# davrempe/contact-human-dynamics

Measured on NVIDIA H100. Metric: optimised frames/sec (batched phys-optim), higher is better.
Workload: dtype f64

## Files before the change

### contact-human-dynamics_b200/csrc/chd_kkt.cu

```cuda
#include <cuda_runtime.h>

#include "chd_block.cuh"
#include "chd_eval.cuh"
#include "chd_kkt_tiles.cuh"

__device__ __forceinline__ void chd_hess_sample(const ChdCtx& c, const ChdKT& K, const int* vk, int s, const ChdSpl* P, const double* sign, int np,
                                                int deriv, double wgt, int lane, double* ws) {
  const bool tau = c.opt_dur && s >= 2 && deriv == 0;
  if (lane < 28) {
    const int pa = lane / 14, q = lane % 14;
    double v0 = 0.0, v1 = 0.0, v2 = 0.0;
    int ia = -1;
    if (pa < np) {
      if (q < 12) {
        const int va = P[pa].var[q];
        const double wa = sign[pa] * chd_slot_w(P[pa], deriv, q);
        if (va >= 0 && wa != 0.0) {
          ia = vk[va];
          v0 = q % 3 == 0 ? wa : 0.0, v1 = q % 3 == 1 ? wa : 0.0, v2 = q % 3 == 2 ? wa : 0.0;
        }
      } else if (tau) {
        ChdTau u;
        chd_spl_tau(c, s, s - 2, P[pa], u);
        const int var = q == 12 ? u.va : u.vb;
        const double* dv = q == 12 ? u.da : u.db;
        if (var >= 0) ia = vk[var], v0 = sign[pa] * dv[0], v1 = sign[pa] * dv[1], v2 = sign[pa] * dv[2];
      }
    }
    ws[lane * 4 + 0] = (double)ia, ws[lane * 4 + 1] = v0, ws[lane * 4 + 2] = v1, ws[lane * 4 + 3] = v2;
  }
  __syncwarp();
  const int ne = np * 14;
  for (int idx = lane; idx < ne * ne; idx += 32) {
    const int a = idx / ne, bq = idx - a * ne;
    const int ia = (int)ws[a * 4], ib = (int)ws[bq * 4];
    if (ia < 0 || ib < 0 || ia < ib) continue;
    const double v = ws[a * 4 + 1] * ws[bq * 4 + 1] + ws[a * 4 + 2] * ws[bq * 4 + 2] + ws[a * 4 + 3] * ws[bq * 4 + 3];
    if (v != 0.0) chd_kadd(K, ia, ib, wgt * v);
  }
  __syncwarp();
}

__device__ void chd_hess_build(const ChdDev& D, int b, const ChdStageDev& sg, double* base, int part, int nparts) {
  const int tid = threadIdx.x, nt = blockDim.x;
  const ChdSeq* h = D.seq + b;
  ChdKT K;
  chd_kt_init(D, h, base, K);
  K.ovf = &D.ipm[b].band_ovf;
  const double sf = D.ipm[b].sf;
  const int* vk = D.var_kkt + (size_t)b * D.n_max;
  ChdCtx c;
  chd_make_ctx(D, b, D.x + (size_t)b * D.n_max, c);
  c.dyn = D.ipm[b].dyn;
  c.opt_dur = sg.opt_dur;
  const int n_ee = h->n_ee, nsp = 2 + n_ee, F = h->F, ns = h->n_smooth;
  __shared__ double s_hws[CHD_THREADS / 32][28 * 4];
  const int lane = tid & 31, warp = tid >> 5, nwarp = nt >> 5;
  for (int it = part * nwarp + warp; it < nsp * F; it += nparts * nwarp) {
    const int s = it / F, i = it % F, cls = s < 2 ? s : 2;
    ChdSpl P[2];
    double sgn[2] = {1.0, -1.0};
    chd_spl_at(c, s, c.t_data[i], P[1]);
    if (sg.w_data[cls] != 0.0) chd_hess_sample(c, K, vk, s, P + 1, sgn, 1, 0, sf * sg.w_data[cls], lane, s_hws[warp]);
    if (i < ns && (sg.w_vel[cls] != 0.0 || sg.w_acc[cls] != 0.0)) {
      chd_spl_at(c, s, c.t_data[i] + h->dt, P[0]);
      if (sg.w_vel[cls] != 0.0) chd_hess_sample(c, K, vk, s, P, sgn, 2, 0, sf * sg.w_vel[cls], lane, s_hws[warp]);
      if (sg.w_acc[cls] != 0.0) chd_hess_sample(c, K, vk, s, P, sgn, 2, 1, sf * sg.w_acc[cls], lane, s_hws[warp]);
    }
  }
  if (part == 0)
    for (int i = K.Na + tid; i < K.Np; i += nt) *chd_kdiag(K, i, true) = 1.0;
  if (part == 0 && !sg.opt_dur && h->dur_band)
    for (int i = tid; i < h->n_dur; i += nt) *chd_kdiag(K, vk[h->dur_xoff[0] + i], true) = 1.0;
  if (part == 0 && sg.opt_dur && sg.w_dur != 0.0) {
    for (int ee = 0; ee < n_ee; ++ee)
      for (int k = tid; k < h->n_phases[ee] - 1; k += nt) {
        const int i = vk[h->dur_xoff[ee] + k];
        chd_kadd(K, i, i, sf * sg.w_dur);
        if (k > 0) {
          const int j = vk[h->dur_xoff[ee] + k - 1];
          chd_kadd(K, j, j, sf * sg.w_dur);
          chd_kadd(K, i, j, -sf * sg.w_dur);
        }
      }
  }
}
__device__ void chd_hess_clear(const ChdDev& D, int b, double* base, int part, int nparts) {
  const size_t cnt2 = D.kstride / 2, per = (cnt2 + nparts - 1) / nparts;
  const size_t lo = (size_t)part * per, hi = lo + per < cnt2 ? lo + per : cnt2;
  double2* dst = reinterpret_cast<double2*>(base);
  for (size_t i = lo + threadIdx.x; i < hi; i += blockDim.x) dst[i] = make_double2(0.0, 0.0);
}
__device__ void chd_rhs_clear(const ChdDev& D, int b) {
  const size_t go = (size_t)b * (D.Na_max + D.nb_max);
  for (int i = threadIdx.x; i < D.Na_max + D.nb_max; i += blockDim.x) D.rhs0[go + i] = 0.0, D.rhs1[go + i] = 0.0;
}

__global__ void __launch_bounds__(CHD_THREADS) chd_k_hess_dur(ChdDev D) {
  const int b = blockIdx.y;
  const ChdIpm& I = D.ipm[b];
  if (I.phase != CHD_PH_RUN || !I.kw_req) return;
  const ChdStageDev sg = D.stages[I.stage];
  if (!sg.opt_dur) return;
  chd_hess_build(D, b, sg, D.Kwork + (size_t)b * D.kstride, blockIdx.x, gridDim.x);
}
__global__ void __launch_bounds__(128) chd_k_hess_fin(ChdDev D, int mode) {
  const int b = blockIdx.x;
  ChdIpm& I = D.ipm[b];
  double* base;
  if (mode == 0) {
    if (I.phase != CHD_PH_BEGIN) return;
    base = D.Kbase + (size_t)b * D.kstride;
  } else {
    if (I.phase != CHD_PH_RUN || !I.kw_req || !D.stages[I.stage].opt_dur) return;
    base = D.Kwork + (size_t)b * D.kstride;
  }
  const ChdSeq* h = D.seq + b;
  const int* vk = D.var_kkt + (size_t)b * D.n_max;
  ChdKT K;
  chd_kt_init(D, h, base, K);
  unsigned char* un = D.unobs + (size_t)b * D.n_max;
  const int mot_lo = h->sp_xoff[2], mot_hi = h->sp_xoff[2 + h->n_ee];
  for (int i = mot_lo + threadIdx.x; i < mot_hi; i += blockDim.x) {
    const int k = vk[i];
    un[i] = k >= 0 && *chd_kdiag(K, k) <= CHD_UNOBS_EPS;
  }
  __syncthreads();
  if (mode == 0 && threadIdx.x == 0) I.phase = CHD_PH_RUN;
}

__device__ __forceinline__ void chd_curv_rows(const ChdDev& D, int b, const ChdKT& K, const ChdStageDev& sg, int wid, int nw, int lane,
                                              double* ws) {
  const ChdSeq* h = D.seq + b;
  const size_t ro = (size_t)b * D.m_max, vo = (size_t)b * D.n_max;
  const int* vk = D.var_kkt + vo;
  ChdCtx c;
  chd_make_ctx(D, b, D.x + vo, c);
  c.dyn = D.ipm[b].dyn;
  c.opt_dur = sg.opt_dur;
  for (int si = 0; si < h->nsets; ++si) {
    const ChdSet st = c.sets[si];
    if (!(sg.set_mask & CHD_MASK(st.type))) continue;
    if (st.type != CHD_SET_ROM && st.type != CHD_SET_HEEL) continue;
    const int nslot = st.type == CHD_SET_ROM ? 38 : 28;
    for (int k = wid; k < st.nitems; k += nw) {
      const int R = st.row0 + k;
      const double yc = D.sc[ro + R] * D.y[ro + R];
      if (!(yc > CHD_CURV_MIN)) continue;
      const double t = c.t_rom[k];
      ChdSpl P0, P1, P2;
      double dRh[3][3];
      if (st.type == CHD_SET_ROM) {
        chd_spl_at(c, 0, t, P0);
        chd_spl_at(c, 1, t, P1);
        chd_spl_at(c, chd_sp_motion(st.a), t, P2);
        double e[3];
        chd_spl_val(c, P1, 0, e);
        ChdTrig tr;
        chd_trig(e, tr);
        const double* hip = chd_hip(c, st.a, t);
        for (int j = 0; j < 3; ++j) {
          double Dj[9];
          chd_dR(tr, j, Dj);
          chd_mv(Dj, hip, dRh[j]);
        }
      } else {
        chd_spl_at(c, chd_sp_motion(st.a), t, P0);
        chd_spl_at(c, chd_sp_motion(st.b), t, P1);
      }
      ChdTau ua, ub;
      ua.va = ua.vb = ub.va = ub.vb = -1;
      if (c.opt_dur) {
        if (st.type == CHD_SET_ROM) chd_spl_tau(c, chd_sp_motion(st.a), st.a, P2, ua);
        else chd_spl_tau(c, chd_sp_motion(st.a), st.a, P0, ua), chd_spl_tau(c, chd_sp_motion(st.b), st.b, P1, ub);
      }
      const int nnode = st.type == CHD_SET_ROM ? 36 : 24;
      for (int a = lane; a < nslot; a += 32) {
        if (a >= nnode) {
          const int t4 = a - nnode;
          const ChdTau& u = t4 < 2 ? ua : ub;
          const int var = (t4 & 1) ? u.vb : u.va;
          const double* dv = (t4 & 1) ? u.db : u.da;
          const int ia = var >= 0 ? vk[var] : -1;
          ws[a * 5 + 0] = (double)ia;
          ws[a * 5 + 1] = ia >= 0 ? (t4 < 2 ? 1.0 : -1.0) : 0.0;
          ws[a * 5 + 2] = ia >= 0 ? dv[0] : 0.0, ws[a * 5 + 3] = ia >= 0 ? dv[1] : 0.0, ws[a * 5 + 4] = ia >= 0 ? dv[2] : 0.0;
          continue;
        }
        const int ba = a / 12, qa = a % 12, da = qa % 3;
        const ChdSpl& Pa = ba == 0 ? P0 : (ba == 1 ? P1 : P2);
        const int va = Pa.var[qa];
        const int ia = va >= 0 ? vk[va] : -1;
        double sgn, v3[3] = {da == 0 ? 1.0 : 0.0, da == 1 ? 1.0 : 0.0, da == 2 ? 1.0 : 0.0};
        if (st.type == CHD_SET_ROM) {
          sgn = ba == 2 ? 1.0 : -1.0;
          if (ba == 1) v3[0] = dRh[da][0], v3[1] = dRh[da][1], v3[2] = dRh[da][2];
        } else {
          sgn = ba == 0 ? 1.0 : -1.0;
        }
        ws[a * 5 + 0] = (double)ia;
        ws[a * 5 + 1] = ia >= 0 ? sgn * chd_slot_w(Pa, 0, qa) : 0.0;
        ws[a * 5 + 2] = v3[0], ws[a * 5 + 3] = v3[1], ws[a * 5 + 4] = v3[2];
      }
      __syncwarp();
      for (int idx = lane; idx < nslot * nslot; idx += 32) {
        const int a = idx / nslot, bq = idx - a * nslot;
        const double wa = ws[a * 5 + 1], wb = ws[bq * 5 + 1];
        if (wa == 0.0 || wb == 0.0) continue;
        const int ia = (int)ws[a * 5], ib = (int)ws[bq * 5];
        if (ia < ib) continue;
        const double dotv = ws[a * 5 + 2] * ws[bq * 5 + 2] + ws[a * 5 + 3] * ws[bq * 5 + 3] + ws[a * 5 + 4] * ws[bq * 5 + 4];
        if (dotv != 0.0) chd_kadd(K, ia, ib, yc * wa * wb * dotv);
      }
      __syncwarp();
    }
  }
}

__global__ void __launch_bounds__(256) chd_k_hess_zero(ChdDev D) {
  const int b = blockIdx.y;
  if (D.ipm[b].phase != CHD_PH_BEGIN) return;
  chd_hess_clear(D, b, D.Kbase + (size_t)b * D.kstride, blockIdx.x, gridDim.x);
  chd_hess_clear(D, b, D.Kwork + (size_t)b * D.kstride, blockIdx.x, gridDim.x);
  if (blockIdx.x == 0) chd_rhs_clear(D, b);
}
__global__ void __launch_bounds__(256, 2) chd_k_hess_base(ChdDev D) {
  __shared__ double s_ws[8][192];
  const int b = blockIdx.y;
  if (D.ipm[b].phase != CHD_PH_BEGIN) return;
  const ChdStageDev sg = D.stages[D.ipm[b].stage];
  ChdKT K;
  chd_kt_init(D, D.seq + b, D.Kwork + (size_t)b * D.kstride, K);
  K.ovf = &D.ipm[b].band_ovf;
  const int warp = threadIdx.x >> 5, nwarp = blockDim.x >> 5;
  chd_curv_rows(D, b, K, sg, blockIdx.x * nwarp + warp, gridDim.x * nwarp, threadIdx.x & 31, s_ws[warp]);
  chd_hess_build(D, b, sg, D.Kbase + (size_t)b * D.kstride, blockIdx.x, gridDim.x);
  chd_hess_build(D, b, sg, D.Kwork + (size_t)b * D.kstride, blockIdx.x, gridDim.x);
}

__device__ __forceinline__ void chd_assemble(const ChdDev& D, int b, const ChdKT& K, double delta_w, double sf, int t0, int tstep,
                                             double* g0, double* g1) {
  const ChdSeq* h = D.seq + b;
  const int n = D.stages[D.ipm[b].stage].opt_dur ? h->n : h->n - h->n_dur;
  const int m = h->m, Na = K.Na;
  const size_t ro = (size_t)b * D.m_max, vo = (size_t)b * D.n_max;
  const int* rf = D.rflag + ro;
  const int* vk = D.var_kkt + vo;
  const int* rk = D.row_kkt + ro;
  const int* ep = D.ent_ptr + (size_t)b * (D.m_max + 1);
  const int* ec = D.ent_col + (size_t)b * D.slots_max;
  const double* Jv = D.Jv + (size_t)b * D.slots_max;
  const double* grad = D.grad + vo;
  auto gidx = [&](int kk) { return kk < Na ? kk : D.Na_max + (kk - Na); };
  auto g_add = [&](int kk, double v0, double v1) {
    atomicAdd(g0 + gidx(kk), v0);
    if (v1 != 0.0) atomicAdd(g1 + gidx(kk), v1);
  };
  const unsigned char* unobs = D.unobs + vo;
  for (int i = t0; i < n; i += tstep) {
    const int k = vk[i];
    if (k < 0) continue;
    if (unobs[i]) chd_kadd(K, k, k, CHD_DW_UNOBS);
    chd_kadd(K, k, k, delta_w);
    g_add(k, -sf * grad[i], 0.0);
  }
  for (int r = t0; r < m; r += tstep) {
    const int f = rf[r];
    const int k = rk[r];
    if (!(f & CHD_ROW_ACTIVE)) {
      if (k >= 0) chd_kadd(K, k, k, -1.0);
      continue;
    }
    const double sc = D.sc[ro + r];
    const int e0 = ep[r], e1 = ep[r + 1];
    if (k >= 0) {
      double diag = -CHD_DELTA_C, rr0, rr1 = 0.0;
      if (f & CHD_ROW_EQ) {
        rr0 = -(sc * D.g[ro + r] - D.dL[ro + r]);
      } else {
        const double s = D.s[ro + r];
        const double gapL = (f & CHD_ROW_HASL) ? s - D.dL[ro + r] : 1.0, gapU = (f & CHD_ROW_HASU) ? D.dU[ro + r] - s : 1.0;
        const double Sig = ((f & CHD_ROW_HASL) ? D.zL[ro + r] / gapL : 0.0) + ((f & CHD_ROW_HASU) ? D.zU[ro + r] / gapU : 0.0);
        diag -= 1.0 / Sig;
        rr0 = -(sc * D.g[ro + r] - s) + D.y[ro + r] / Sig;
        rr1 = (((f & CHD_ROW_HASL) ? 1.0 / gapL : 0.0) - ((f & CHD_ROW_HASU) ? 1.0 / gapU : 0.0)) / Sig;
      }
      chd_kadd(K, k, k, diag);
      g_add(k, rr0, rr1);
      const double ys = sc * D.y[ro + r];
      for (int e = e0; e < e1; ++e) {
        const int col = ec[e];
        if (col < 0) continue;
        const int kc = vk[col];
        if (kc < 0) continue;
        const double jv = Jv[e];
        if (jv == 0.0) continue;
        chd_kadd(K, k, kc, sc * jv);
        g_add(kc, -ys * jv, 0.0);
      }
    } else {
      const double s = D.s[ro + r];
      const double gapL = (f & CHD_ROW_HASL) ? s - D.dL[ro + r] : 1.0, gapU = (f & CHD_ROW_HASU) ? D.dU[ro + r] - s : 1.0;
      const double Sig = ((f & CHD_ROW_HASL) ? D.zL[ro + r] / gapL : 0.0) + ((f & CHD_ROW_HASU) ? D.zU[ro + r] / gapU : 0.0);
      const double coef0 = Sig * (sc * D.g[ro + r] - s);
      const double beta = ((f & CHD_ROW_HASL) ? 1.0 / gapL : 0.0) - ((f & CHD_ROW_HASU) ? 1.0 / gapU : 0.0);
      for (int ea = e0; ea < e1; ++ea) {
        const int ca = ec[ea];
        if (ca < 0) continue;
        const int ka = vk[ca];
        if (ka < 0) continue;
        const double va = sc * Jv[ea];
        if (va == 0.0) continue;
        g_add(ka, -va * coef0, va * beta);
        for (int eb = e0; eb < e1; ++eb) {
          const int cb = ec[eb];
          if (cb < 0) continue;
          const int kb = vk[cb];
          if (kb < 0 || ka < kb) continue;
          const double vb = sc * Jv[eb];
          if (vb != 0.0) chd_kadd(K, ka, kb, Sig * va * vb);
        }
      }
    }
  }
}

struct ChdKktCtx {
  int b, tid, nt, lane, warp, nwarp;
  ChdIpm* I;
  ChdStageDev sg;
  const ChdSeq* h;
  int n, m, n_act, Qs, Q, nbt, nbp8, nbl, nbc, NBR, nbt_s;
  size_t ro, vo, n_even, xs_len, win_region;
  const int *rf, *vk, *rk, *ep, *ec;
  const double *Jv, *grad;
  ChdKT K;
  double *red, *cc, *ypan, *xpan, *dinv, *win, *bwin, *vecn, *xs, *xs2;
  double sf, mu, tau, delta_w;
  bool polish;
};

template <bool WS>
__device__ __forceinline__ void chd_kkt_ctx_init(const ChdDev& D, ChdIpm& I, ChdKktCtx& c) {
  extern __shared__ double sm[];
  const int b = blockIdx.x;
  c.b = b, c.I = &I;
  c.sg = D.stages[I.stage];
  const ChdSeq* h = c.h = D.seq + b;
  c.n = h->n, c.m = h->m, c.tid = threadIdx.x, c.nt = blockDim.x;
  c.lane = c.tid & 31, c.warp = c.tid >> 5, c.nwarp = c.nt >> 5;
  c.ro = (size_t)b * D.m_max, c.vo = (size_t)b * D.n_max;
  c.rf = D.rflag + c.ro;
  c.vk = D.var_kkt + c.vo;
  c.rk = D.row_kkt + c.ro;
  c.ep = D.ent_ptr + (size_t)b * (D.m_max + 1);
  c.ec = D.ent_col + (size_t)b * D.slots_max;
  c.Jv = D.Jv + (size_t)b * D.slots_max;
  c.grad = D.grad + c.vo;
  ChdKT& K = c.K;
  chd_kt_init(D, h, D.Kwork + (size_t)b * D.kstride, K);
  K.ovf = &I.band_ovf;
  if (!c.sg.opt_dur) K.q = D.Qfix - 1;
  c.n_act = c.sg.opt_dur ? c.n : c.n - h->n_dur;
  c.Qs = K.Q, c.Q = c.sg.opt_dur ? K.Q : D.Qfix, c.nbt = K.nbt, c.nbp8 = K.nbp8, c.nbl = c.sg.opt_dur ? h->nb : h->nb_fix, c.nbc = K.nbc;
  c.NBR = c.nbl, c.nbt_s = (c.nbl + 1 + 7) >> 3;
  c.n_even = (size_t)((D.n_max + 1) & ~1), c.xs_len = (size_t)(8 * D.nbc_max + c.nbp8);
  double* gs = WS ? nullptr : D.scratch + (size_t)b * D.scratch_stride;
  c.red = sm;
  c.cc = c.red + CHD_KKT_THREADS;
  c.ypan = c.cc + c.nbp8 * c.nbp8;
  c.xpan = c.ypan + (c.Q + c.nbt) * 64;
  c.dinv = c.ypan + D.pan_doubles;
  c.win_region = (size_t)D.win_tiles * 64 + (size_t)c.Qs * c.nbt * 64;
  c.win = WS ? c.dinv + 16 : gs + c.n_even + c.xs_len + 8 * (size_t)D.nbc_max;
  c.bwin = c.win + (size_t)D.win_tiles * 64;
  c.vecn = WS ? c.win + c.win_region - c.n_even : gs;
  c.xs = WS ? c.vecn - c.xs_len : c.vecn + c.n_even;
  c.xs2 = WS ? c.ypan : c.xs + c.xs_len;
  c.sf = I.sf;
}

__device__ __forceinline__ bool chd_kkt_errors(const ChdDev& D, ChdKktCtx& c, int& s_fail) {
  ChdIpm& I = *c.I;
  const int b = c.b, tid = c.tid, nt = c.nt, n = c.n, m = c.m, n_act = c.n_act;
  const size_t ro = c.ro, vo = c.vo;
  const int *rf = c.rf, *vk = c.vk, *ep = c.ep, *ec = c.ec;
  const double *Jv = c.Jv, *grad = c.grad, sf = c.sf;
  double* red = c.red;
  double mu = I.mu;
  const int* erow = D.ent_row + (size_t)b * D.slots_max;
  const int* cptr = D.col_ptr + (size_t)b * (D.n_max + 1);
  const int* cent = D.col_ent + (size_t)b * D.slots_max;
  double* rowv = D.dy + ro;
  double a_ysum = 0, a_zsum = 0, a_cviol = 0, a_theta = 0, a_rs = 0, a_cmax = -INFINITY, a_cmin = INFINITY, a_violu = 0;
  for (int r = tid; r < m; r += nt) {
    const int f = rf[r];
    if (!(f & CHD_ROW_ACTIVE)) {
      rowv[r] = 0.0;
      continue;
    }
    const double sc = D.sc[ro + r], gval = D.g[ro + r], d = sc * gval, y = D.y[ro + r];
    a_ysum += fabs(y);
    a_violu = fmax(a_violu, fmax(D.row_lo[ro + r] - gval, gval - D.row_hi[ro + r]));
    rowv[r] = sc * y;
    if (f & CHD_ROW_EQ) {
      const double re = d - D.dL[ro + r];
      a_cviol = fmax(a_cviol, fabs(re));
      a_theta += fabs(re);
    } else {
      const double s = D.s[ro + r], ri = d - s, zL = D.zL[ro + r], zU = D.zU[ro + r];
      a_cviol = fmax(a_cviol, fabs(ri));
      a_theta += fabs(ri);
      a_rs = fmax(a_rs, fabs(-y - zL + zU));
      a_zsum += zL + zU;
      if (f & CHD_ROW_HASL) { const double cp = (s - D.dL[ro + r]) * zL; a_cmax = fmax(a_cmax, cp); a_cmin = fmin(a_cmin, cp); }
      if (f & CHD_ROW_HASU) { const double cp = (D.dU[ro + r] - s) * zU; a_cmax = fmax(a_cmax, cp); a_cmin = fmin(a_cmin, cp); }
    }
  }
  __syncthreads();
  double a_dual = 0;
  if (!I.dyn) {
    for (int i = tid; i < n_act; i += nt) {
      double v = sf * grad[i];
      for (int t = cptr[i]; t < cptr[i + 1]; ++t) {
        const int e = cent[t];
        v += rowv[erow[e]] * Jv[e];
      }
      if (vk[i] >= 0) a_dual = fmax(a_dual, fabs(v));
    }
  } else {
    double* jty = D.jty + vo;
    for (int i = tid; i < n; i += nt) jty[i] = 0.0;
    __syncthreads();
    for (int r = tid; r < m; r += nt) {
      const double ys = rowv[r];
      if (ys == 0.0) continue;
      for (int e = ep[r]; e < ep[r + 1]; ++e) {
        const int col = ec[e];
        if (col >= 0 && Jv[e] != 0.0) atomicAdd(jty + col, ys * Jv[e]);
      }
    }
    __syncthreads();
    for (int i = tid; i < n_act; i += nt)
      if (vk[i] >= 0) a_dual = fmax(a_dual, fabs(sf * grad[i] + jty[i]));
  }
  const double ysum = chd_block_sum(a_ysum, red), zsum = chd_block_sum(a_zsum, red);
  const double cviol = chd_block_max(a_cviol, red), theta = chd_block_sum(a_theta, red);
  const double dual_inf = fmax(chd_block_max(a_dual, red), chd_block_max(a_rs, red));
  const double cmax = chd_block_max(a_cmax, red), cmin = chd_block_min(a_cmin, red);
  const double violu = fmax(chd_block_max(a_violu, red), 0.0);
  const int nbnd = I.n_bounds;
  const double s_d = fmax(CHD_S_MAX, (ysum + zsum) / fmax((double)(I.m_act + nbnd), 1.0)) / CHD_S_MAX;
  const double s_c = fmax(CHD_S_MAX, zsum / fmax((double)nbnd, 1.0)) / CHD_S_MAX;
  auto compl_err = [&](double mm) { return nbnd > 0 ? fmax(fabs(cmax - mm), fabs(cmin - mm)) : 0.0; };
  const double E0 = fmax(fmax(dual_inf / s_d, cviol), compl_err(0.0) / s_c);
  const double dual_u = dual_inf / sf, compl_u = compl_err(0.0) / sf;
  bool done = false;
  int new_status = 1;
  if (E0 <= CHD_TOL && violu <= CHD_CONSTR_VIOL_TOL && dual_u <= CHD_DUAL_INF_TOL && compl_u <= CHD_COMPL_INF_TOL) new_status = 0, done = true;
  else if (I.iter >= I.max_iter) new_status = -1, done = true;
  if (!done) {
    const double mu_min = fmin(CHD_TOL, CHD_COMPL_INF_TOL) / (CHD_KAPPA_EPS + 1.0);
    while (true) {
      const double Emu = fmax(fmax(dual_inf / s_d, cviol), compl_err(mu) / s_c);
      if (Emu <= CHD_KAPPA_EPS * mu && mu > mu_min) mu = fmax(mu_min, fmin(CHD_KAPPA_MU * mu, pow(mu, CHD_THETA_MU)));
      else break;
    }
  }
  __syncthreads();
  if (tid == 0) {
    I.f = D.cost[2 * b];
    I.E0 = E0, I.viol_u = violu, I.dual_u = dual_u, I.compl_u = compl_u;
    I.status = new_status;
    s_fail = 0;
    if (done) chd_stage_advance(D, I, new_status, c.sg.snap_after);
    if (!done) {
      I.mu = mu;
      I.tau = fmax(CHD_TAU_MIN, 1.0 - mu);
      if (I.iter == 0) I.theta_max = 1e4 * fmax(1.0, theta), I.theta_min = 1e-4 * fmax(1.0, theta), I.theta_ref = theta;
      if (mu != I.mu_filter) I.nfilt = 0, I.mu_filter = mu;
      I.theta0 = theta;
    }
  }
  if (done) return true;
  c.mu = mu;
  c.tau = fmax(CHD_TAU_MIN, 1.0 - mu);
  c.polish = E0 <= CHD_TOL && dual_u <= CHD_DUAL_INF_TOL && compl_u <= CHD_COMPL_INF_TOL && violu > CHD_CONSTR_VIOL_TOL &&
             I.delta_w < CHD_DW_POLISH;
  c.delta_w = c.polish ? CHD_DW_POLISH : I.delta_w;
  return false;
}

__device__ __forceinline__ void chd_kkt_assemble(const ChdDev& D, const ChdKktCtx& c) {
  const ChdIpm& I = *c.I;
  const ChdKT& K = c.K;
  const int tid = c.tid, nt = c.nt, n_act = c.n_act, nbl = c.nbl, nbt = c.nbt, nbp8 = c.nbp8, NBR = c.NBR, Na = K.Na;
  const int* vk = c.vk;
  const double mu = c.mu;
  if (c.polish) {
    const double extra = c.delta_w - I.delta_w;
    for (int i = tid; i < n_act; i += nt)
      if (vk[i] >= 0) chd_kadd(K, vk[i], vk[i], extra);
  }
  const double* r0 = D.rhs0 + (size_t)c.b * (D.Na_max + D.nb_max);
  const double* r1 = D.rhs1 + (size_t)c.b * (D.Na_max + D.nb_max);
  for (int i = tid; i < K.Np; i += nt)
    K.bord[((size_t)(i >> 3) * nbt + (NBR >> 3)) * 64 + (NBR & 7) * 8 + (i & 7)] = i < Na ? r0[i] + mu * r1[i] : 0.0;
  for (int i = tid; i < nbl; i += nt) K.corn[(size_t)NBR * nbp8 + i] = r0[D.Na_max + i] + mu * r1[D.Na_max + i];
}

template <class BandTile, class BordTile>
__device__ __forceinline__ void chd_kkt_update_block(const ChdKktCtx& c, const int* gi, const int* gj, const bool* vi, const bool* vj, bool diag,
                                                     int GB, const BandTile& band_tile, const BordTile& bord_tile) {
  const int lane = c.lane;
  const double2 z = make_double2(0.0, 0.0);
  double2 xf[2], yf[2];
#pragma unroll
  for (int a = 0; a < 2; ++a) {
    xf[a] = vi[a] ? *reinterpret_cast<const double2*>(c.xpan + gi[a] * 64 + 2 * lane) : z;
    yf[a] = vj[a] ? *reinterpret_cast<const double2*>(c.ypan + gj[a] * 64 + 2 * lane) : z;
  }
  double* Cp[4];
  double2 cv[4];
#pragma unroll
  for (int t = 0; t < 4; ++t) {
    const int a = t & 1, cl = t >> 1;
    bool ok = vi[a] && vj[cl] && !(diag && a == 0 && cl == 1);
    ok = ok && !(gi[a] == 0 && gj[cl] == 0);
    Cp[t] = nullptr;
    if (ok) {
      if (gi[a] < GB) Cp[t] = band_tile(gi[a], gj[cl]) + (lane >> 2) * 8 + 2 * (lane & 3);
      else if (gj[cl] < GB) Cp[t] = bord_tile(gi[a] - GB, gj[cl]) + (lane >> 2) * 8 + 2 * (lane & 3);
      else Cp[t] = c.cc + (size_t)((gi[a] - GB) * 8 + (lane >> 2)) * c.nbp8 + (gj[cl] - GB) * 8 + 2 * (lane & 3);
    }
    cv[t] = ok ? *reinterpret_cast<const double2*>(Cp[t]) : z;
  }
  const double2 xt = make_double2(-xf[0].x, -xf[0].y), xb = make_double2(-xf[1].x, -xf[1].y);
#pragma unroll
  for (int cl = 0; cl < 2; ++cl) chd_mma_16x8x8(cv[2 * cl], cv[2 * cl + 1], xt, xb, yf[cl]);
#pragma unroll
  for (int t = 0; t < 4; ++t)
    if (Cp[t]) *reinterpret_cast<double2*>(Cp[t]) = cv[t];
}

template <class BandTile, class BordTile>
__device__ __forceinline__ void chd_kkt_update_compact(const ChdKktCtx& c, const unsigned short* s_pairs, unsigned char* cmp, const int* gnz,
                                                       int GB, int Gm, int tq, const BandTile& band_tile, const BordTile& bord_tile) {
  const int lane = c.lane, warp = c.warp;
  int na;
  {
    const int g1 = lane + 32;
    const bool act0 = lane < Gm && (lane >= GB || lane < tq) && gnz[lane];
    const bool act1 = g1 < Gm && (g1 >= GB || g1 < tq) && gnz[g1 < 96 ? g1 : 0];
    const unsigned m0 = __ballot_sync(0xffffffffu, act0), m1 = __ballot_sync(0xffffffffu, act1);
    const unsigned below = (1u << lane) - 1u;
    const int n0 = __popc(m0);
    na = n0 + __popc(m1);
    if (act0) cmp[__popc(m0 & below)] = (unsigned char)lane;
    if (act1) cmp[n0 + __popc(m1 & below)] = (unsigned char)g1;
    __syncwarp();
  }
  const int step = c.nwarp - 1;
  const int nb2 = (na + 1) >> 1, nblk = nb2 * (nb2 + 1) / 2;
  for (int p = warp - 1; p < nblk; p += step) {
    const int bi = s_pairs[p] >> 8, bj = s_pairs[p] & 255;
    const int i1 = 2 * bi + 1, j1 = 2 * bj + 1;
    const int gi[2] = {cmp[2 * bi], cmp[i1 & 63]}, gj[2] = {cmp[2 * bj], cmp[j1 & 63]};
    const bool vi[2] = {true, i1 < na}, vj[2] = {true, j1 < na};
    chd_kkt_update_block(c, gi, gj, vi, vj, bi == bj, GB, band_tile, bord_tile);
  }
}

template <class BandTile, class BordTile>
__device__ __forceinline__ void chd_kkt_update_wide(const ChdKktCtx& c, const unsigned short* s_pairs, const int* gnz, int GB, int Gm,
                                                    int tq, const BandTile& band_tile, const BordTile& bord_tile) {
  auto live = [&](int g) { return g < Gm && (g >= GB || g < tq) && gnz[g]; };
  const int nb2 = (Gm + 1) >> 1, nblk = nb2 * (nb2 + 1) / 2;
  for (int p = c.warp - 1; p < nblk; p += c.nwarp - 1) {
    const int bi = s_pairs[p] >> 8, bj = s_pairs[p] & 255;
    const int gi[2] = {2 * bi, 2 * bi + 1}, gj[2] = {2 * bj, 2 * bj + 1};
    const bool vi[2] = {live(gi[0]), live(gi[1])}, vj[2] = {live(gj[0]), live(gj[1])};
    if (!(vi[0] || vi[1]) || !(vj[0] || vj[1])) continue;
    chd_kkt_update_block(c, gi, gj, vi, vj, bi == bj, GB, band_tile, bord_tile);
  }
}

template <bool WS>
__device__ __forceinline__ void chd_kkt_factor(const ChdKktCtx& c, int& s_fail) {
  const ChdKT& K = c.K;
  const int tid = c.tid, nt = c.nt, lane = c.lane, warp = c.warp, nwarp = c.nwarp;
  const int Qs = c.Qs, Q = c.Q, nbt = c.nbt, nbp8 = c.nbp8, nbc = c.nbc, nbt_s = c.nbt_s;
  double *cc = c.cc, *ypan = c.ypan, *xpan = c.xpan, *dinv = c.dinv, *win = c.win, *bwin = c.bwin;
  for (int i = tid; i < nbp8 * nbp8; i += nt) cc[i] = K.corn[i];
  if (WS) {
    for (int idx = tid; idx < Q * Q * 64; idx += nt) {
      const int e = idx & 63, pr = idx >> 6, J = pr / Q, t = pr % Q;
      if (J + t < Q && J < nbc && J + t < nbc) win[chd_win_slot(J + t, J, Q) * 64 + e] = K.band[((size_t)J * Qs + t) * 64 + e];
    }
    for (int idx = tid; idx < Q * nbt * 64; idx += nt) {
      const int J = idx / (nbt * 64);
      if (J < nbc) bwin[idx] = K.bord[(size_t)J * nbt * 64 + idx % (nbt * 64)];
    }
  }
  __syncthreads();
  __shared__ int s_rs[2][96];
  __shared__ int s_gnz[2][96];
  constexpr int kPairs = WS ? 3000 : CHD_KKT_GROUPS_MAX * (CHD_KKT_GROUPS_MAX + 1) / 2;
  __shared__ unsigned short s_pairs[kPairs];
  __shared__ unsigned char s_cmp[CHD_KKT_THREADS / 32][64];
  __shared__ __align__(16) double s_winv[2][64];
#ifdef CHD_PROFILE
  __shared__ unsigned long long s_upd_end;
  double prof_diag = 0.0, prof_upd = 0.0;
  if (tid == 0) s_upd_end = 0;
#endif
  const int GB = K.q, Gm = K.q + nbt_s, nb2 = (Gm + 1) >> 1, npairs = nb2 * (nb2 + 1) / 2;
  for (int p = tid; p < npairs && p < kPairs; p += nt) {
    int gi = (int)((sqrt(8.0 * p + 1.0) - 1.0) * 0.5);
    while (gi * (gi + 1) / 2 > p) --gi;
    while ((gi + 1) * (gi + 2) / 2 <= p) ++gi;
    s_pairs[p] = (unsigned short)((gi << 8) | (p - gi * (gi + 1) / 2));
  }
  auto tri = [](int a_, int b_) { return a_ > b_ ? a_ * (a_ + 1) / 2 + b_ : b_ * (b_ + 1) / 2 + a_; };
  for (int g = tid; g < GB; g += nt) s_rs[0][g] = (1 + g) % Q;
  for (int g = tid; g < 96; g += nt) s_gnz[0][g] = 0, s_gnz[1][g] = 0;
  if (warp == 0) {
    const bool ok = chd_tile_ldl(WS ? win : K.band, dinv, s_winv[0], lane);
    if (!ok && lane == 0) s_fail = 1;
  }
  __syncthreads();
  int kslot = 0, cur = 0;
  for (int Kc = 0; Kc < nbc; ++Kc, cur ^= 1) {
    const int tq = min(K.q, nbc - 1 - Kc);
    const int* rs = s_rs[cur];
    auto band_tile = [&](int gi, int gj) -> double* {
      return WS ? win + (size_t)tri(rs[gi], rs[gj]) * 64 : K.band + ((size_t)(Kc + 1 + gj) * Qs + (gi - gj)) * 64;
    };
    auto bord_tile = [&](int bi, int gj) -> double* {
      return WS ? bwin + ((size_t)rs[gj] * nbt + bi) * 64 : K.bord + ((size_t)(Kc + 1 + gj) * nbt + bi) * 64;
    };
    double* Tkk = WS ? win + (size_t)tri(kslot, kslot) * 64 : K.band + (size_t)Kc * Qs * 64;
    double* Bk = WS ? bwin + (size_t)kslot * nbt * 64 : K.bord + (size_t)Kc * nbt * 64;
    const double* dv = dinv + 8 * cur;
    {
      const double* wv = s_winv[cur];
      const int r = lane >> 2, k = lane & 3, ng = tq + nbt_s;
      const double2 wf = *reinterpret_cast<const double2*>(wv + 2 * lane);
      const double d0 = dv[2 * k], d1 = dv[2 * k + 1];
      const int f0 = r * 8 + chd_frag_col(2 * k), f1 = r * 8 + chd_frag_col(2 * k + 1);
      for (int g0 = 2 * warp; g0 < ng; g0 += 2 * nwarp) {
        double2 a[2], y[2];
#pragma unroll
        for (int h = 0; h < 2; ++h) {
          const int g = g0 + h;
          const double* A = g < tq ? (WS ? win + (size_t)tri(rs[g], kslot) * 64 : K.band + ((size_t)Kc * Qs + 1 + g) * 64) : Bk + (g - tq) * 64;
          a[h] = g < ng ? make_double2(A[r * 8 + k], A[r * 8 + k + 4]) : make_double2(0.0, 0.0);
          y[h] = make_double2(0.0, 0.0);
        }
        chd_mma_16x8x8(y[0], y[1], a[0], a[1], wf);
#pragma unroll
        for (int h = 0; h < 2; ++h) {
          const int g = g0 + h;
          if (g >= ng) break;
          const bool band_t = g < tq;
          const int pg = band_t ? g : GB + (g - tq);
          const double x0 = y[h].x * d0, x1 = y[h].y * d1;
          ypan[pg * 64 + f0] = y[h].x, ypan[pg * 64 + f1] = y[h].y;
          xpan[pg * 64 + f0] = x0, xpan[pg * 64 + f1] = x1;
          double* G = band_t ? K.band + ((size_t)Kc * Qs + 1 + g) * 64 : K.bord + ((size_t)Kc * nbt + (g - tq)) * 64;
          *reinterpret_cast<double2*>(G + r * 8 + 2 * k) = make_double2(x0, x1);
          const bool nz = __any_sync(0xffffffffu, x0 != 0.0 || x1 != 0.0);
          if (lane == 0 && nz) s_gnz[cur][pg] = 1;
        }
      }
    }
    if (WS)
      for (int e = tid; e < 64; e += nt) K.band[(size_t)Kc * Qs * 64 + e] = Tkk[e];
    __syncthreads();
    const int In = Kc + Q;
#ifdef CHD_PROFILE
    const long long tc0 = clock64();
#endif
    if (WS && In < nbc) {
      for (int idx = tid - 32; idx < Q * 32 + nbt_s * 32; idx += nt - 32) {
        if (idx < 0) break;
        const int tile = idx >> 5, off = (idx & 31) * 2;
        if (tile < Q) {
          const int J = tile < GB ? Kc + 1 + tile : In;
          double* dst = tile < GB ? win + (size_t)tri(kslot, rs[tile]) * 64 : Tkk;
          chd_copy16(dst + off, K.band + ((size_t)J * Qs + (In - J)) * 64 + off, WS);
        } else {
          chd_copy16(Bk + (tile - Q) * 64 + off, K.bord + (size_t)In * nbt * 64 + (tile - Q) * 64 + off, WS);
        }
      }
    }
    if (warp == 0) {
      if (tq >= 1) {
        double* Tn = band_tile(0, 0);
        chd_tile_sub_xyT(Tn, xpan, ypan, lane);
        __syncwarp();
        const bool ok = chd_tile_ldl(Tn, dinv + 8 * (cur ^ 1), s_winv[cur ^ 1], lane);
        if (!ok && lane == 0) s_fail = 1;
      }
#ifdef CHD_PROFILE
      if (lane == 0) prof_diag += (double)(clock64() - tc0);
#endif
    } else {
      if (warp == 1) {
        for (int g = lane; g < GB; g += 32) {
          int v = kslot + 2 + g;
          while (v >= Q) v -= Q;
          s_rs[cur ^ 1][g] = v;
        }
        for (int g = lane; g < Gm; g += 32) s_gnz[cur ^ 1][g] = 0;
      }
      if (!WS && Gm > 64) chd_kkt_update_wide(c, s_pairs, s_gnz[cur], GB, Gm, tq, band_tile, bord_tile);
      else chd_kkt_update_compact(c, s_pairs, s_cmp[warp], s_gnz[cur], GB, Gm, tq, band_tile, bord_tile);
#ifdef CHD_PROFILE
      if (lane == 0) atomicMax(&s_upd_end, (unsigned long long)clock64());
#endif
    }
    chd_copy_wait(WS);
    __syncthreads();
#ifdef CHD_PROFILE
    if (tid == 0) prof_upd += (double)((long long)s_upd_end - tc0);
#endif
    kslot = kslot + 1 == Q ? 0 : kslot + 1;
  }
#ifdef CHD_PROFILE
  if (tid == 0) c.I->prof[6] += prof_diag, c.I->prof[7] += prof_upd;
#endif
}

__device__ __forceinline__ void chd_kkt_border(const ChdDev& D, const ChdKktCtx& c, int& s_fail) {
  const int tid = c.tid, nt = c.nt, lane = c.lane, warp = c.warp, nbl = c.nbl, nbp8 = c.nbp8, NBR = c.NBR, Na = c.K.Na;
  double* cc = c.cc;
  for (int k = 0; k < nbl; ++k) {
    const double dk = cc[k * nbp8 + k];
    if (tid == 0 && !(dk > 0.0 && isfinite(dk))) s_fail = 1;
    __syncthreads();
    const double ik = 1.0 / dk;
    const int rem = nbl - k - 1;
    for (int idx = tid; idx < rem * rem; idx += nt) {
      const int i = k + 1 + idx / rem, j = k + 1 + idx % rem;
      if (j <= i) cc[i * nbp8 + j] -= cc[i * nbp8 + k] * ik * cc[j * nbp8 + k];
    }
    for (int j = k + 1 + tid; j < nbl; j += nt) cc[NBR * nbp8 + j] -= cc[j * nbp8 + k] * ik * cc[NBR * nbp8 + k];
    __syncthreads();
  }
  double* xb = c.xs + 8 * D.nbc_max;
  if (warp == 0) {
    for (int j = lane; j < nbl; j += 32) xb[j] = cc[NBR * nbp8 + j];
    __syncwarp();
    for (int k = nbl - 1; k >= 0; --k) {
      const double xk = xb[k] / cc[k * nbp8 + k];
      __syncwarp();
      for (int j = lane; j < k; j += 32) xb[j] -= cc[k * nbp8 + j] * xk;
      if (lane == 0) xb[k] = xk;
      __syncwarp();
    }
  }
  __syncthreads();
  for (int i = tid; i < nbl; i += nt) D.sol[(size_t)c.b * (D.Na_max + D.nb_max) + Na + i] = xb[i];
}

template <bool WS>
__device__ __forceinline__ void chd_kkt_backsub(const ChdDev& D, const ChdKktCtx& c) {
  const ChdKT& K = c.K;
  const int tid = c.tid, nt = c.nt, lane = c.lane, warp = c.warp, Q = c.Q, Qs = c.Qs, nbt = c.nbt, nbl = c.nbl, nbc = c.nbc;
  const int NBR = c.NBR, Na = K.Na;
  double *xs = c.xs, *sol = D.sol + (size_t)c.b * (D.Na_max + D.nb_max);
  const double* xb = xs + 8 * D.nbc_max;
  double* accv = c.xs2;
  for (int i = tid; i < K.Np; i += nt) {
    const double* bt = K.bord + (size_t)(i >> 3) * nbt * 64 + (i & 7);
    double v = bt[NBR * 8];
    for (int q2 = 0; q2 < nbl; ++q2) v -= bt[q2 * 8] * xb[q2];
    accv[i] = v;
  }
  const int per = Q * 64;
  const int R = max(1, (int)((c.win_region - (WS ? c.n_even + c.xs_len : 0)) / 64) / (2 * Q));
  double* stg = c.win;
  auto stage_chunk = [&](int Ktop, int buf, int t0, int tstep) {
    for (int idx = t0; idx < R * Q * 32; idx += tstep) {
      const int rr = idx / (Q * 32), rem = idx - rr * (Q * 32);
      const int Kr = Ktop - rr;
      if (Kr < 0) break;
      const int tile = rem >> 5, off = (rem & 31) * 2;
      const int J = tile == 0 ? Kr : Kr - tile;
      if (J < 0) continue;
      chd_copy16(stg + ((size_t)buf * R + rr) * per + tile * 64 + off, K.band + ((size_t)J * Qs + (Kr - J)) * 64 + off, WS);
    }
  };
  stage_chunk(nbc - 1, 0, tid, nt);
  chd_copy_wait(WS);
  __syncthreads();
  int buf = 0;
  for (int Ktop = nbc - 1; Ktop >= 0; Ktop -= R, buf ^= 1) {
    if (warp != 0) {
      stage_chunk(Ktop - R, buf ^ 1, tid - 32, nt - 32);
    } else {
      for (int rr = 0; rr < R && Ktop - rr >= 0; ++rr) {
        const int Kc = Ktop - rr;
        const double* T0 = stg + ((size_t)buf * R + rr) * per;
        double xk[8];
#pragma unroll
        for (int cl = 7; cl >= 0; --cl) {
          double v = accv[Kc * 8 + cl];
#pragma unroll
          for (int p = 7; p > cl; --p) v -= T0[p * 8 + cl] * xk[p];
          xk[cl] = v;
        }
        if (lane < 8) {
          const int gi = Kc * 8 + lane;
          double v = xk[0];
#pragma unroll
          for (int cl = 1; cl < 8; ++cl) v = lane == cl ? xk[cl] : v;
          xs[gi] = v;
          if (gi < Na) sol[gi] = v;
        }
        const int nrow = min(K.q, Kc);
        for (int idx = lane; idx < nrow * 8; idx += 32) {
          const int g = idx >> 3, cl = idx & 7;
          const double* T = T0 + (g + 1) * 64;
          double v = 0.0;
#pragma unroll
          for (int r = 0; r < 8; ++r) v += T[r * 8 + cl] * xk[r];
          accv[(Kc - 1 - g) * 8 + cl] -= v;
        }
        __syncwarp();
      }
    }
    chd_copy_wait(WS);
    __syncthreads();
  }
}

__device__ __forceinline__ bool chd_kkt_no_step(const ChdDev& D, const ChdKktCtx& c, const int& s_fail) {
  ChdIpm& I = *c.I;
  const int tid = c.tid, nt = c.nt, n = c.n, m = c.m;
  const size_t ro = c.ro, vo = c.vo;
  if (I.band_ovf) {
    __syncthreads();
    if (tid == 0) I.status = -2, chd_stage_advance(D, I, -2, c.sg.snap_after);
    return true;
  }
  if (s_fail) {
    if (tid == 0) {
      I.delta_w = fmin(fmax(I.delta_w * 100.0, 1e-4), CHD_DW_MAX * 10);
      I.a_pr = 0.0, I.a_du = 0.0, I.dphi = 0.0;
      I.ls_fail += 1;
      I.step_ready = 1;
      I.kw_req = 1;
      if (I.delta_w > CHD_DW_MAX) I.status = -2, chd_stage_advance(D, I, -2, c.sg.snap_after);
    }
    for (int i = tid; i < n; i += nt) D.dx[vo + i] = 0.0;
    for (int r = tid; r < m; r += nt) D.ds[ro + r] = 0.0, D.dy[ro + r] = 0.0, D.dzL[ro + r] = 0.0, D.dzU[ro + r] = 0.0;
    return true;
  }
  return false;
}

__device__ __forceinline__ void chd_kkt_recover(const ChdDev& D, const ChdKktCtx& c) {
  ChdIpm& I = *c.I;
  const ChdSeq* h = c.h;
  const int b = c.b, tid = c.tid, nt = c.nt, n = c.n, m = c.m, n_act = c.n_act;
  const size_t ro = c.ro, vo = c.vo;
  const int *rf = c.rf, *vk = c.vk, *rk = c.rk, *ep = c.ep, *ec = c.ec;
  const double *Jv = c.Jv, *grad = c.grad, *sol = D.sol + (size_t)c.b * (D.Na_max + D.nb_max), sf = c.sf, mu = c.mu, tau = c.tau;
  double *vecn = c.vecn, *red = c.red;
  double* dx = D.dx + vo;
  for (int i = tid; i < n; i += nt) {
    const int k = vk[i];
    const double v = (k >= 0 && i < n_act) ? sol[k] : 0.0;
    dx[i] = v;
    vecn[i] = v;
  }
  __syncthreads();
  if (c.sg.opt_dur) {
    for (int ee = 0; ee < h->n_ee; ++ee)
      for (int k = 1 + tid; k < h->n_phases[ee] - 1; k += nt) dx[h->dur_xoff[ee] + k] = vecn[h->dur_xoff[ee] + k] - vecn[h->dur_xoff[ee] + k - 1];
  }
  double a_pr = 1.0, a_du = 1.0, a_dphi = 0.0, a_phi = 0.0;
  for (int i = tid; i < n; i += nt) a_dphi += sf * grad[i] * vecn[i];
  for (int r = tid; r < m; r += nt) {
    const int f = rf[r];
    if (!(f & CHD_ROW_ACTIVE)) continue;
    if (f & CHD_ROW_EQ) {
      D.dy[ro + r] = sol[rk[r]];
      D.ds[ro + r] = 0.0;
      continue;
    }
    const double sc = D.sc[ro + r], s = D.s[ro + r];
    double Jdx = 0.0;
    for (int e = ep[r]; e < ep[r + 1]; ++e) {
      const int col = ec[e];
      if (col >= 0) Jdx += Jv[e] * vecn[col];
    }
    const double riq = sc * D.g[ro + r] - s;
    const double ds = sc * Jdx + riq;
    const bool hl = f & CHD_ROW_HASL, hu = f & CHD_ROW_HASU;
    const double gapL = hl ? s - D.dL[ro + r] : 1.0, gapU = hu ? D.dU[ro + r] - s : 1.0;
    const double zL = D.zL[ro + r], zU = D.zU[ro + r];
    const double sigL = hl ? zL / gapL : 0.0, sigU = hu ? zU / gapU : 0.0;
    const double bvec = (hl ? mu / gapL : 0.0) - (hu ? mu / gapU : 0.0);
    const double dy = (sigL + sigU) * ds - D.y[ro + r] - bvec;
    const double dzL = hl ? mu / gapL - zL - sigL * ds : 0.0;
    const double dzU = hu ? mu / gapU - zU + sigU * ds : 0.0;
    D.ds[ro + r] = ds, D.dy[ro + r] = dy, D.dzL[ro + r] = dzL, D.dzU[ro + r] = dzU;
    if (hl && ds < 0) a_pr = fmin(a_pr, -tau * gapL / ds);
    if (hu && ds > 0) a_pr = fmin(a_pr, tau * gapU / ds);
    if (hl && dzL < 0) a_du = fmin(a_du, -tau * zL / dzL);
    if (hu && dzU < 0) a_du = fmin(a_du, -tau * zU / dzU);
    if (hl) a_dphi -= mu * ds / gapL, a_phi -= mu * log(gapL);
    if (hu) a_dphi += mu * ds / gapU, a_phi -= mu * log(gapU);
  }
  a_pr = chd_block_min(a_pr, red);
  a_du = chd_block_min(a_du, red);
  const double dphi = chd_block_sum(a_dphi, red);
  const double phib = chd_block_sum(a_phi, red);
  if (tid == 0) {
    I.a_pr = a_pr, I.a_du = a_du, I.dphi = dphi;
    I.phi0 = sf * D.cost[2 * b] + phib;
    I.step_ready = 1;
    I.kw_req = 1;
  }
}

template <bool WS>
__device__ __forceinline__ void chd_kkt_body(const ChdDev& D) {
  __shared__ int s_fail;
  ChdIpm& I = D.ipm[blockIdx.x];
  if (I.phase != CHD_PH_RUN) return;
  ChdKktCtx c;
  chd_kkt_ctx_init<WS>(D, I, c);
#ifdef CHD_PROFILE
  long long tk0 = clock64();
#define CHD_PROF(slot) do { __syncthreads(); if (c.tid == 0) { long long t_ = clock64(); I.prof[slot] += (double)(t_ - tk0); tk0 = t_; } } while (0)
#else
#define CHD_PROF(slot) do { } while (0)
#endif
  if (chd_kkt_errors(D, c, s_fail)) return;
  CHD_PROF(0);
  chd_kkt_assemble(D, c);
  __syncthreads();
  CHD_PROF(1);
  chd_kkt_factor<WS>(c, s_fail);
  CHD_PROF(2);
  chd_kkt_border(D, c, s_fail);
  CHD_PROF(3);
  chd_kkt_backsub<WS>(D, c);
  CHD_PROF(4);
  if (chd_kkt_no_step(D, c, s_fail)) return;
  __syncthreads();
  chd_kkt_recover(D, c);
  CHD_PROF(5);
}
#undef CHD_PROF

__global__ void __launch_bounds__(256) chd_k_kcopy(ChdDev D) {
  const int b = blockIdx.y;
  if (!D.ipm[b].kw_req) return;
  if (blockIdx.x == 0) chd_rhs_clear(D, b);
  if (D.stages[D.ipm[b].stage].opt_dur && D.ipm[b].phase == CHD_PH_RUN) {
    chd_hess_clear(D, b, D.Kwork + (size_t)b * D.kstride, blockIdx.x, gridDim.x);
    return;
  }
  const size_t cnt2 = D.kstride / 2, per = (cnt2 + gridDim.x - 1) / gridDim.x;
  const size_t lo = (size_t)blockIdx.x * per, hi = lo + per < cnt2 ? lo + per : cnt2;
  const double2* src = reinterpret_cast<const double2*>(D.Kbase + (size_t)b * D.kstride);
  double2* dst = reinterpret_cast<double2*>(D.Kwork + (size_t)b * D.kstride);
  const size_t nt = blockDim.x;
  size_t i = lo + threadIdx.x;
  for (; i + 3 * nt < hi; i += 4 * nt) {
    const double2 v0 = src[i], v1 = src[i + nt], v2 = src[i + 2 * nt], v3 = src[i + 3 * nt];
    dst[i] = v0, dst[i + nt] = v1, dst[i + 2 * nt] = v2, dst[i + 3 * nt] = v3;
  }
  for (; i < hi; i += nt) dst[i] = src[i];
}

__global__ void __launch_bounds__(256) chd_k_curv(ChdDev D) {
  __shared__ double s_ws[8 * 192];
  const int b = blockIdx.y;
  const ChdIpm& I = D.ipm[b];
  if (!I.kw_req || I.phase != CHD_PH_RUN) return;
  ChdKT K;
  chd_kt_init(D, D.seq + b, D.Kwork + (size_t)b * D.kstride, K);
  K.ovf = &D.ipm[b].band_ovf;
  const int warp = threadIdx.x >> 5, lane = threadIdx.x & 31;
  chd_curv_rows(D, b, K, D.stages[I.stage], blockIdx.x * 8 + warp, gridDim.x * 8, lane, s_ws + warp * 192);
}

__global__ void __launch_bounds__(256) chd_k_asm(ChdDev D) {
  const int b = blockIdx.y;
  const ChdIpm& I = D.ipm[b];
  if (I.phase != CHD_PH_RUN) return;
  ChdKT K;
  chd_kt_init(D, D.seq + b, D.Kwork + (size_t)b * D.kstride, K);
  K.ovf = &D.ipm[b].band_ovf;
  if (!D.stages[I.stage].opt_dur) K.q = D.Qfix - 1;
  const size_t go = (size_t)b * (D.Na_max + D.nb_max);
  chd_assemble(D, b, K, I.delta_w, I.sf, blockIdx.x * blockDim.x + threadIdx.x, gridDim.x * blockDim.x, D.rhs0 + go, D.rhs1 + go);
}

__global__ void __launch_bounds__(256) chd_k_fp64_peak(int mode, int iters, double* sink) {
  const double s = 1.0 + 1e-9 * threadIdx.x;
  double2 a[8];
#pragma unroll
  for (int i = 0; i < 8; ++i) a[i] = make_double2(0.5 + i, 1.5 + i);
  if (mode == 0) {
    for (int it = 0; it < iters; ++it) {
#pragma unroll
      for (int i = 0; i < 8; ++i) a[i].x = fma(a[i].x, s, 1e-3);
    }
  } else {
    const double2 x = make_double2(s, s), y = make_double2(1.0 - 1e-9 * threadIdx.x, 1.0);
    for (int it = 0; it < iters; ++it) {
#pragma unroll
      for (int i = 0; i < 4; ++i) chd_mma_16x8x8(a[2 * i], a[2 * i + 1], x, x, y);
    }
  }
  double t = 0;
#pragma unroll
  for (int i = 0; i < 8; ++i) t += a[i].x + a[i].y;
  if (t == 123.456) sink[threadIdx.x] = t;
}

__global__ void __launch_bounds__(CHD_KKT_THREADS) chd_k_kkt(ChdDev D) { chd_kkt_body<true>(D); }
__global__ void __launch_bounds__(CHD_KKT_THREADS) chd_k_kkt_gwin(ChdDev D) { chd_kkt_body<false>(D); }
```

Before: 13770.

## Block the border Cholesky into 8x8 tiles with tensor-core MMA and pad backsub staging

Replaces the scalar right-looking border factorisation, which needs two block barriers per column, with a blocked LDL over 8x8 tiles. Warp 0 factors the next diagonal tile while the other warps apply the trailing update, and the panel solve uses f64 MMA fragments. The border back-solve now expects unit-diagonal factors. Backsub staging tiles are padded to a 72-double stride to cut shared-memory bank conflicts, and the off-diagonal accumulation processes four tile rows per lane for more ILP. The new code depends on extra context buffers (ypan, xpan, dinv, red, nwarp) and adds more shared-memory use and complexity.

```diff
diff --git a/contact-human-dynamics_b200/csrc/chd_kkt.cu b/contact-human-dynamics_b200/csrc/chd_kkt.cu
--- a/contact-human-dynamics_b200/csrc/chd_kkt.cu
+++ b/contact-human-dynamics_b200/csrc/chd_kkt.cu
@@ -733,35 +733,100 @@
 }
 
 __device__ __forceinline__ void chd_kkt_border(const ChdDev& D, const ChdKktCtx& c, int& s_fail) {
-  const int tid = c.tid, nt = c.nt, lane = c.lane, warp = c.warp, nbl = c.nbl, nbp8 = c.nbp8, NBR = c.NBR, Na = c.K.Na;
-  double* cc = c.cc;
-  for (int k = 0; k < nbl; ++k) {
-    const double dk = cc[k * nbp8 + k];
-    if (tid == 0 && !(dk > 0.0 && isfinite(dk))) s_fail = 1;
+  const int tid = c.tid, lane = c.lane, warp = c.warp, nwarp = c.nwarp, nbl = c.nbl, nbp8 = c.nbp8, NBR = c.NBR, Na = c.K.Na;
+  double *cc = c.cc, *ypan = c.ypan, *xpan = c.xpan, *dinv = c.dinv;
+  double* winv = c.red;
+  double* Td = c.red + 128;
+  const int nbb = (nbl + 7) >> 3, nT = (NBR >> 3) + 1;
+  auto diag_tile = [&](int kb, int slot, bool upd) {
+    double* T = cc + (size_t)8 * kb * (nbp8 + 1);
+    for (int e = lane; e < 64; e += 32) {
+      const int r = e >> 3, col = e & 7, row = 8 * kb + r;
+      double v = T[r * nbp8 + col];
+      if (!upd && row >= nbl) v = r == col ? 1.0 : (row == NBR && col < r ? v : 0.0);
+      Td[e] = v;
+    }
+    __syncwarp();
+    if (upd) {
+      chd_tile_sub_xyT(Td, xpan, ypan, lane);
+      __syncwarp();
+      for (int e = lane; e < 64; e += 32) {
+        const int r = e >> 3, col = e & 7, row = 8 * kb + r;
+        if (row >= nbl && col <= r) Td[e] = r == col ? 1.0 : (row == NBR ? Td[e] : 0.0);
+      }
+      __syncwarp();
+    }
+    chd_tile_ldl(Td, dinv + 8 * slot, winv + 64 * slot, lane);
+    __syncwarp();
+    if (lane < 8 && 8 * kb + lane < nbl) {
+      const double dk = Td[lane * 9];
+      if (!(dk > 0.0 && isfinite(dk))) s_fail = 1;
+    }
+    for (int e = lane; e < 64; e += 32)
+      if ((e & 7) <= (e >> 3)) T[(e >> 3) * nbp8 + (e & 7)] = Td[e];
+    __syncwarp();
+  };
+  if (warp == 0 && nbb > 0) diag_tile(0, 0, false);
+  __syncthreads();
+  for (int kb = 0, cur = 0; kb < nbb; ++kb, cur ^= 1) {
+    const int ng = nT - 1 - kb;
+    {
+      const int r = lane >> 2, k = lane & 3;
+      const double2 wf = *reinterpret_cast<const double2*>(winv + 64 * cur + 2 * lane);
+      const double* dv = dinv + 8 * cur;
+      const double d0 = dv[2 * k], d1 = dv[2 * k + 1];
+      const int f0 = r * 8 + chd_frag_col(2 * k), f1 = r * 8 + chd_frag_col(2 * k + 1);
+      for (int g0 = 2 * warp; g0 < ng; g0 += 2 * nwarp) {
+        double2 a[2], y[2];
+#pragma unroll
+        for (int h = 0; h < 2; ++h) {
+          const double* A = cc + (size_t)(8 * (kb + 1 + g0 + h) + r) * nbp8 + 8 * kb;
+          a[h] = g0 + h < ng ? make_double2(A[k], A[k + 4]) : make_double2(0.0, 0.0);
+          y[h] = make_double2(0.0, 0.0);
+        }
+        chd_mma_16x8x8(y[0], y[1], a[0], a[1], wf);
+#pragma unroll
+        for (int h = 0; h < 2; ++h) {
+          const int g = g0 + h;
+          if (g >= ng) break;
+          const double x0 = y[h].x * d0, x1 = y[h].y * d1;
+          ypan[g * 64 + f0] = y[h].x, ypan[g * 64 + f1] = y[h].y;
+          xpan[g * 64 + f0] = x0, xpan[g * 64 + f1] = x1;
+          *reinterpret_cast<double2*>(cc + (size_t)(8 * (kb + 1 + g) + r) * nbp8 + 8 * kb + 2 * k) = make_double2(x0, x1);
+        }
+      }
+    }
     __syncthreads();
-    const double ik = 1.0 / dk;
-    const int rem = nbl - k - 1;
-    for (int idx = tid; idx < rem * rem; idx += nt) {
-      const int i = k + 1 + idx / rem, j = k + 1 + idx % rem;
-      if (j <= i) cc[i * nbp8 + j] -= cc[i * nbp8 + k] * ik * cc[j * nbp8 + k];
-    }
-    for (int j = k + 1 + tid; j < nbl; j += nt) cc[NBR * nbp8 + j] -= cc[j * nbp8 + k] * ik * cc[NBR * nbp8 + k];
+    if (warp == 0) {
+      if (kb + 1 < nbb) diag_tile(kb + 1, cur ^ 1, true);
+    } else {
+      ChdKktCtx cs = c;
+      cs.cc = cc + (size_t)8 * (kb + 1) * (nbp8 + 1);
+      auto none = [](int, int) -> double* { return nullptr; };
+      const int nb2 = (ng + 1) >> 1, nblk = nb2 * (nb2 + 1) / 2;
+      for (int p = warp - 1; p < nblk; p += nwarp - 1) {
+        int bi = 0;
+        while ((bi + 1) * (bi + 2) / 2 <= p) ++bi;
+        const int bj = p - bi * (bi + 1) / 2;
+        const int gi[2] = {2 * bi, 2 * bi + 1}, gj[2] = {2 * bj, 2 * bj + 1};
+        const bool vi[2] = {true, 2 * bi + 1 < ng}, vj[2] = {true, 2 * bj + 1 < ng};
+        chd_kkt_update_block(cs, gi, gj, vi, vj, bi == bj, 0, none, none);
+      }
+    }
     __syncthreads();
   }
   double* xb = c.xs + 8 * D.nbc_max;
   if (warp == 0) {
     for (int j = lane; j < nbl; j += 32) xb[j] = cc[NBR * nbp8 + j];
     __syncwarp();
-    for (int k = nbl - 1; k >= 0; --k) {
-      const double xk = xb[k] / cc[k * nbp8 + k];
+    for (int k = nbl - 1; k > 0; --k) {
+      const double xk = xb[k];
+      for (int j = lane; j < k; j += 32) xb[j] -= cc[k * nbp8 + j] * xk;
       __syncwarp();
-      for (int j = lane; j < k; j += 32) xb[j] -= cc[k * nbp8 + j] * xk;
-      if (lane == 0) xb[k] = xk;
-      __syncwarp();
     }
   }
   __syncthreads();
-  for (int i = tid; i < nbl; i += nt) D.sol[(size_t)c.b * (D.Na_max + D.nb_max) + Na + i] = xb[i];
+  for (int i = tid; i < nbl; i += c.nt) D.sol[(size_t)c.b * (D.Na_max + D.nb_max) + Na + i] = xb[i];
 }
 
 template <bool WS>
@@ -778,8 +843,9 @@
     for (int q2 = 0; q2 < nbl; ++q2) v -= bt[q2 * 8] * xb[q2];
     accv[i] = v;
   }
-  const int per = Q * 64;
-  const int R = max(1, (int)((c.win_region - (WS ? c.n_even + c.xs_len : 0)) / 64) / (2 * Q));
+  constexpr int TS = 72;
+  const int per = Q * TS;
+  const int R = max(1, (int)((c.win_region - (WS ? c.n_even + c.xs_len : 0)) / per) / 2);
   double* stg = c.win;
   auto stage_chunk = [&](int Ktop, int buf, int t0, int tstep) {
     for (int idx = t0; idx < R * Q * 32; idx += tstep) {
@@ -789,7 +855,7 @@
       const int tile = rem >> 5, off = (rem & 31) * 2;
       const int J = tile == 0 ? Kr : Kr - tile;
       if (J < 0) continue;
-      chd_copy16(stg + ((size_t)buf * R + rr) * per + tile * 64 + off, K.band + ((size_t)J * Qs + (Kr - J)) * 64 + off, WS);
+      chd_copy16(stg + ((size_t)buf * R + rr) * per + tile * TS + off, K.band + ((size_t)J * Qs + (Kr - J)) * 64 + off, WS);
     }
   };
   stage_chunk(nbc - 1, 0, tid, nt);
@@ -819,14 +885,19 @@
           xs[gi] = v;
           if (gi < Na) sol[gi] = v;
         }
-        const int nrow = min(K.q, Kc);
-        for (int idx = lane; idx < nrow * 8; idx += 32) {
-          const int g = idx >> 3, cl = idx & 7;
-          const double* T = T0 + (g + 1) * 64;
-          double v = 0.0;
-#pragma unroll
-          for (int r = 0; r < 8; ++r) v += T[r * 8 + cl] * xk[r];
-          accv[(Kc - 1 - g) * 8 + cl] -= v;
+        const int nrow = min(K.q, Kc), cl = lane & 7;
+        for (int g0 = lane >> 3; g0 < nrow; g0 += 16) {
+          double v[4];
+#pragma unroll
+          for (int j = 0; j < 4; ++j) {
+            const double* T = T0 + (min(g0 + 4 * j, nrow - 1) + 1) * TS;
+            v[j] = 0.0;
+#pragma unroll
+            for (int r = 0; r < 8; ++r) v[j] += T[r * 8 + cl] * xk[r];
+          }
+#pragma unroll
+          for (int j = 0; j < 4; ++j)
+            if (g0 + 4 * j < nrow) accv[(Kc - 1 - g0 - 4 * j) * 8 + cl] -= v[j];
         }
         __syncwarp();
       }
```

Measured after the change: 14120 (median of 6 runs). 2.5% higher.
